# tmr4/T41_SDR

Hardware: AMD Instinct MI355X
Metric: MSamples/s I/Q through full RX chain, batch=4096; achieved HBM GB/s vs roofline (higher is better)
Workload: dtype f32; 1 GPU; configs[1]: batched SSB (USB 200-3000 Hz) RX chain, decimate-by-8 + 512-pt fast-conv + demod + interpolate-by-8, 4096 channels x 2048 complex f32 samples per frame per GPU, per-channel NCO, AGC off, 128 consecutive frames per channel per launch; batch=4096, frame_len=2048, fft_length=512, frames_per_launch=128, buffer_layout=channel-major, world_size_observed=1

## Files before the change

t41_sdr_amd/csrc/rx512_kernel.hpp:

```cpp
#pragma once
#include "rx_chains.hpp"

namespace t41 {

template <int PART, bool AGC = false>
struct Geo {
  static constexpr bool kResident = (PART == 0) && !AGC;
  static constexpr int kWaves = kResident ? 16 : 4;
  static constexpr int kTab = kResident ? 1024 : kLdsTabFloats;
  static constexpr int kTw1 = kResident ? 0 : kLdsTabTw1;
  static constexpr int kTw2 = kResident ? 448 : kLdsTabTw2;
  static constexpr int kSlice = kResident ? 2496 : kLdsFloatsPerWave;
  static constexpr int kTotal = kTab + kWaves * kSlice;
  static constexpr int kX = 0;
  static constexpr int kXF = kResident ? 1348 : kXFloats;
  static constexpr int kY1 = kXF;
  static constexpr int kOV = kY1 + kY1Floats;
  static constexpr int kH1 = kOV + 512;
  static constexpr int kScr = kResident ? 80 : 0;
  static constexpr int kI1 = kScr;
};
template <int MODE, int PART, bool AGC, bool PIPE>
using Rx512Geo = Geo<PART, geo4(MODE, AGC) && !PIPE>;
static_assert(!Geo<0>::kResident || Geo<0>::kTotal * sizeof(float) == 160 * 1024, "PART 0: one workgroup owns the CU's LDS");
static_assert(Geo<1>::kTotal * sizeof(float) == 40960, "PART 1/2: four workgroups per CU");
static_assert(pipe_layout(7).counters == (size_t)7 * kPipeSlots * kPipeSlotFloats * sizeof(float) &&
              pipe_layout(7).timeout == pipe_layout(7).counters + ((size_t)7 + 15) * 16 * sizeof(unsigned long long) &&
              pipe_layout(7).second == pipe_layout(7).counters + ((size_t)7 + 16) * 32 * sizeof(float) && kPipeStatWords == 16,
              "rx512_kernel's pipe_err / pipe_stat / sam_slots arithmetic follows pipe_layout()");
static_assert(!Geo<0>::kResident || (Geo<0>::kH1 + 24 <= Geo<0>::kSlice && Geo<0>::kScr + 8 * kFftRow * 2 <= Geo<0>::kXF &&
                                     Geo<0>::kI1 + 284 <= Geo<0>::kXF && Geo<0>::kScr >= 68), "resident LDS layout");

constexpr int kPartMap = 4;
constexpr int kPartSet = 8;
constexpr int kPartA24 = 16;
constexpr int kPartOut = 32;
template <int MODE, bool DEBUG, int PARTM, bool PLAIN, bool AGC = false, bool WQ15 = false, bool SEGPAR = false, bool PIPE = false>
__global__ __launch_bounds__((Rx512Geo<MODE, (PARTM & 3), AGC, PIPE>::kWaves * 64), 4) void rx512_kernel(const RxArgs a) {
  T41RX_CLK_BEGIN();
  constexpr int PART = PARTM & 3;
  constexpr bool MAP = (PARTM & kPartMap) != 0;
  constexpr bool SET = (PARTM & kPartSet) != 0;
  constexpr bool A24 = (PARTM & kPartA24) != 0;
  constexpr bool OUT = (PARTM & kPartOut) != 0;
  static_assert(PART <= 2 && (PARTM & ~(3 | kPartMap | kPartSet | kPartA24 | kPartOut)) == 0,
                "PARTM = PART, PART + kPartMap, or PART + kPartMap + kPartSet, each of the mapped ones with or without kPartA24 and kPartOut");
  static_assert(!OUT || (MAP && PART == 0 && !DEBUG && !SEGPAR) || ((PARTM & ~kPartSet) == 2 + kPartOut && SEGPAR),
                "the output-map form is a twin of the mapped FFT_LENGTH 512 kernels without taps, and of the segment-parallel back kernel");
  static_assert(!A24 || (MAP && PART == 0 && !DEBUG && !SEGPAR), "the 24 kS/s form is a twin of the mapped FFT_LENGTH 512 kernels without taps");
  static_assert(!SET || (MAP && PART == 0 && !SEGPAR) || (PARTM == 2 + kPartOut + kPartSet && SEGPAR),
                "the set form is a twin of the mapped FFT_LENGTH 512 kernels, and of the back kernel's output-map form");
  static_assert(!MAP || PART != 2, "the back end of the long-FFT pipeline reads no antenna samples");
  static_assert(!SEGPAR || (PART == 1 && MODE != kModeNfm) || (PART == 2 && MODE == kModeSsb && !AGC), "SEGPAR variants");
  static_assert(!PIPE || ((AGC || MODE == kModeSam) && PART == 0 && !DEBUG && !SEGPAR),
                "PIPE: the pipelined variants -- AGC on (see agc_prep_pipe), the synchronous detector with the AGC off (sam_chain_pipe), or both (PSA)");
  constexpr bool PSAM = PIPE && MODE == kModeSam && !AGC;
  constexpr bool PSA = PIPE && MODE == kModeSam && AGC;
  constexpr int kPF = PSAM ? kPrefetchPipeSam : PIPE ? kPrefetchPipe : kPrefetch;
  typedef Rx512Geo<MODE, PART, AGC, PIPE> G;
  constexpr bool KEEP = G::kResident;
  constexpr int NW = G::kWaves;
  constexpr int kX = G::kX, kY1 = G::kY1, kScr = G::kScr, kI1 = G::kI1;
  __shared__ __attribute__((aligned(16))) float smem[G::kTotal];
  constexpr int L = 2048, D = 256, N = 512;
  const int seg = (PART == 0) ? 1 : a.seg;
  const size_t state_stride = state_floats(512 * seg);
  int lane = threadIdx.x & 63;
  const int wv = __builtin_amdgcn_readfirstlane(threadIdx.x >> 6);
  const int job = blockIdx.x * NW + wv;
  const int runs = SEGPAR ? (a.nframes + a.seg_run - 1) / a.seg_run : 1;
  const int ch = SEGPAR ? job / runs : job;
  const int seg0 = SEGPAR ? (job - ch * runs) * a.seg_run : 0;
  const int seg1 = SEGPAR ? (seg0 + a.seg_run < a.nframes ? seg0 + a.seg_run : a.nframes) : a.nframes;

  auto stage_tables = [&]() {
    const float4 *src = reinterpret_cast<const float4 *>(a.tab);
    float4 *dst = reinterpret_cast<float4 *>(smem);
    if (PART == 1) {
      if (threadIdx.x < 128) dst[threadIdx.x] = reinterpret_cast<const float4 *>(a.tab + kTabSinCos)[threadIdx.x];
    } else if (KEEP) {
      if (threadIdx.x < 224) dst[threadIdx.x] = src[kTabTw1 / 2 + threadIdx.x];
      else if (threadIdx.x >= 256 && threadIdx.x < 256 + 56)
        reinterpret_cast<float2 *>(smem)[G::kTw2 + threadIdx.x - 256] =
            a.tab[kTabTw2 + 64 * ((threadIdx.x - 256) >> 3) + ((threadIdx.x - 256) & 7)];
      else if (PIPE && threadIdx.x >= 320 && threadIdx.x < 332)
        reinterpret_cast<unsigned *>(smem)[kPipeFlags + threadIdx.x - 320] = 0u;
    } else if (MODE == kModeSam) {
      for (int i = threadIdx.x; i < 516; i += 256) smem[i] = reinterpret_cast<const float *>(a.tab + kTabSam)[i];
      for (int i = 512 / 2 + threadIdx.x; i < (512 + 448) / 2; i += 256) dst[i] = src[i];
      if (threadIdx.x < 56)
        reinterpret_cast<float2 *>(smem)[kLdsTabTw2 + threadIdx.x] = a.tab[kTabTw2 + 64 * (threadIdx.x >> 3) + (threadIdx.x & 7)];
    } else {
      for (int i = threadIdx.x; i < (512 + 448) / 2; i += 256) dst[i] = src[i];
      if (threadIdx.x < 56)
        reinterpret_cast<float2 *>(smem)[kLdsTabTw2 + threadIdx.x] = a.tab[kTabTw2 + 64 * (threadIdx.x >> 3) + (threadIdx.x & 7)];
    }
    __syncthreads();
  };
  const float2 hp8 = a.tab[kTabHp8 + lane];
  const float2 hp4 = a.tab[kTabHp4 + lane];
  if (ch >= a.nchan) {
    if (PART != 2) stage_tables();
    return;
  }

  const cf *ltab = reinterpret_cast<const cf *>(smem);
  float *lds = smem + G::kTab + wv * G::kSlice;
  float *st = a.state + (size_t)ch * state_stride;
  typedef const __attribute__((address_space(4))) int *MapPtr;
  const int pset = SET ? ((MapPtr)a.set_of)[ch] : 0;
  const CoefPtr cf0 = SET ? (CoefPtr)a.coef + pset : (CoefPtr)a.coef;
  const NcoPtr nco = (NcoPtr)(a.nco + ch);
  const float2 *__restrict__ tab = a.tab;
// ... 669 lines not shown
          wave_sync();
  #pragma unroll
          for (int rd = 0; rd < 2; ++rd) {
            const int m0 = 128 * rd + 2 * lane;
            f2 acc = splat(0.0f);
            float tp[96];
  #pragma unroll
            for (int c = 0; c < 96; c += 16) {
              float chunk[16];
              load_taps<16>(chunk, (CFloatPtr)cf0, kCoDeemph + c);
  #pragma unroll
              for (int k = 0; k < 16; ++k) tp[c + k] = chunk[k];
  #pragma unroll
              for (int jj = c / 2; jj < c / 2 + 8; ++jj) {
                if (2 * jj > kDeemphTaps) continue;
                const float2 w = *reinterpret_cast<const float2 *>(ds + m0 + 2 * jj);
                static_assert(kDeemphTaps == 81, "2 jj <= 80 below: tap 2 jj always exists");
                const float t_m1 = (jj > 0) ? tp[2 * jj - 1] : 0.0f;
                const float t_p1 = (2 * jj + 1 < kDeemphTaps) ? tp[2 * jj + 1] : 0.0f;
                f2 pr = f2{tp[2 * jj], t_m1} * splat(w.x);
                acc = acc + pr;
                pr = f2{t_p1, tp[2 * jj]} * splat(w.y);
                acc = acc + pr;
              }
            }
            au[rd][0] = (m0 < D - kDeemphTaps) ? acc.x : y2[rd][0].y;
            au[rd][1] = (m0 + 1 < D - kDeemphTaps) ? acc.y : y2[rd][1].y;
          }
          wave_sync();
        }
        if (PART == 0) {
          if (lane == 63) *reinterpret_cast<cf *>(st + kStMisc + kMiscNfmI) = y2[0][1];
        } else {
          if (lane == 63 && (f & (seg - 1)) == seg / 2 - 1) *reinterpret_cast<cf *>(st + kStMisc + kMiscNfmI) = y2[1][1];
          nfm_carry = cf{__int_as_float(__builtin_amdgcn_readlane(__float_as_int(y2[1][1].x), 63)),
                         __int_as_float(__builtin_amdgcn_readlane(__float_as_int(y2[1][1].y), 63))};
        }
  #pragma unroll
        for (int rd = 0; rd < 2; ++rd)
  #pragma unroll
          for (int e = 0; e < 2; ++e) y2[rd][e] = cf{au[rd][e], 0.0f};
      }
      if (PART == 1) {
        float *mid = a.mid + ((size_t)ch * a.nframes + f) * (2 * D);
  #pragma unroll
        for (int rd = 0; rd < 2; ++rd)
          *reinterpret_cast<float4 *>(mid + 2 * (128 * rd + 2 * lane)) =
              make_float4(y2[rd][0].x, y2[rd][0].y, y2[rd][1].x, y2[rd][1].y);
        continue;
      }


      {
        cf *tb = reinterpret_cast<cf *>(lds + kScr);
  #pragma unroll
        for (int rd = 0; rd < 2; ++rd)
          *reinterpret_cast<float4 *>(lds + kScr + 2 * (128 * rd + 2 * lane)) =
              make_float4(y2[rd][0].x, y2[rd][0].y, y2[rd][1].x, y2[rd][1].y);
        wave_sync();
  #pragma unroll
        for (int j = 0; j < 4; ++j) v[4 + j] = tb[lane + 64 * j];
        constexpr bool OVL_REAL = MODE == kModeNfm;
        if (KEEP) {
          cf *ov = reinterpret_cast<cf *>(lds + G::kOV);
  #pragma unroll
          for (int j = 0; j < 4; ++j) v[j] = ov[64 * j + lane];
  #pragma unroll
          for (int j = 0; j < 4; ++j) {
            if (OVL_REAL) ov[64 * j + lane].x = v[4 + j].x;
            else ov[64 * j + lane] = v[4 + j];
          }
        } else {
          cf *ov = reinterpret_cast<cf *>(st + kStOverlap);
  #pragma unroll
          for (int j = 0; j < 4; ++j) {
            if (OVL_REAL) ov[64 * j + lane].x = v[4 + j].x;
            else ov[64 * j + lane] = v[4 + j];
          }
        }
        if (OVL_REAL) {
  #pragma unroll
          for (int j = 0; j < 4; ++j) v[j].y = 0.0f;
        }
      }

      STAMP(6);
      FRESH_LANE();
      {
        cf tw1[7], tw2[7];
        cf mk[8];
        constexpr bool GMASK = KEEP || MODE == kModeSam;
        constexpr bool SMASK = SET && !GMASK;
        if (SMASK) {
  #pragma unroll
          for (int r = 0; r < 8; ++r) {
            const float2 t = ptab[kTabMask + 64 * r + lane];
            mk[r] = cf{t.x, t.y};
          }
        }
        if (!GMASK) {
  #pragma unroll
          for (int q = 0; q < 7; ++q) {
            tw1[q] = ltab[G::kTw1 + 64 * q + lane];
            tw2[q] = ltab[G::kTw2 + 8 * q + (lane & 7)];
          }
        }
        if (GMASK) {
          fft512_ldstw<false>(v, ltab + G::kTw1 + lane, ltab + G::kTw2 + (lane & 7), lds + kScr, lane, [&]() {
  #pragma unroll
            for (int r = 0; r < 8; ++r) {
              const float2 t = ptab[kTabMask + 64 * r + lane];
              mk[r] = cf{t.x, t.y};
            }
          });
        } else {
          fft512<false>(v, tw1, tw2, lds + kScr, lane);
        }
  #pragma unroll
        for (int r = 0; r < 8; ++r) v[r] = cmul(v[r], (GMASK || SMASK) ? mk[r] : ltab[kLdsTabMask + 64 * r + lane]);
        if (DEBUG && a.spect_max && tap_row >= 0) {
          float *sp = a.spect ? a.spect + ((size_t)ch * tap_stride + tap_row) * 1024 : nullptr;
          float best = -1.0f;
          int besti = 0;
  #pragma unroll
          for (int r = 0; r < 8; ++r) {
            const int k = lane + 64 * r;
            const float re = v[r].x * 512.0f, im = v[r].y * 512.0f;
            const float e0 = im * im, e1 = re * re;
            if (sp) *reinterpret_cast<float2 *>(sp + 1022 - 2 * k) = make_float2(e0, e1);
            if (e1 >= best) { best = e1; besti = 1023 - 2 * k; }
            if (e0 >= best) { best = e0; besti = 1022 - 2 * k; }
          }
  #pragma unroll
          for (int m = 1; m < 64; m <<= 1) {
            const float ob = __shfl_xor(best, m, 64);
            const int oi = __shfl_xor(besti, m, 64);
            if (ob > best || (ob == best && oi < besti)) { best = ob; besti = oi; }
          }
          if (lane == 0) {
            float *mx = a.spect_max + ((size_t)ch * tap_stride + tap_row) * 3;
            const float ave = (float)(.5 * (double)best + .5 * (double)st[kStMisc + kMiscMaxSqAve]);
            mx[0] = best;
            mx[1] = (float)besti;
            mx[2] = ave;
            st[kStMisc + kMiscMaxSqAve] = ave;
          }
        }
        if (GMASK)
          fft512_ldstw<true>(v, ltab + G::kTw1 + lane, ltab + G::kTw2 + (lane & 7), lds + kScr, lane, []() {});
        else
          fft512<true>(v, tw1, tw2, lds + kScr, lane);
      }
    }
    FRESH_LANE();
    if (PART != 2 || LONGC) {
      const float fixed_gain = fresh_coef(cf0)->sc[kScFixedGain];
      cf og[4];
      if (PSA) {
        const int left = a.nchan - NW * (int)blockIdx.x;
        const int nvalid = left < NW ? left : NW;
        unsigned *fa = reinterpret_cast<unsigned *>(smem) + kPipeFlags;
        unsigned *fs = fa + 5;
        unsigned *pipe_err = reinterpret_cast<unsigned *>(reinterpret_cast<unsigned long long *>(a.agc_pipe + (size_t)a.nchan * kPipeSlots * kPipeSlotFloats) +
                                                          ((size_t)a.nchan + 15) * 16);
        float *sam_slots = a.agc_pipe + (size_t)a.nchan * kPipeSlots * kPipeSlotFloats + ((size_t)a.nchan + 16) * 32;
        const size_t ch0 = (size_t)NW * blockIdx.x;
        auto claim = [&](unsigned *word, int g) -> bool {
          unsigned won = 0u;
          if (lane == 0) {
            unsigned expect = (unsigned)g;
            won = __hip_atomic_compare_exchange_strong(word, &expect, (unsigned)(g + 1), __ATOMIC_RELAXED, __ATOMIC_RELAXED, __HIP_MEMORY_SCOPE_WORKGROUP) ? 1u : 0u;
          }
          return __builtin_amdgcn_readfirstlane(won) != 0u;
        };
        static_assert(!PSA || (NW == 16 && kScr + kPipeStageFloats <= G::kXF && kScr + kPipeSamStageFloats <= G::kXF), "chain staging inside the X scratch");
        if (f < seg1) {
          float *pslot = a.agc_pipe + ((size_t)ch * kPipeSlots + f % kPipeSlots) * kPipeSlotFloats;
          if (first_iter) agmag = make_float2(agc_mag(cf{agrec.x, agrec.y}), agc_mag(cf{agrec.z, agrec.w}));
          agrec = agc_prep_pipe<AgcLds<true>, true>(v, agrec, agmag, lds, pslot, cf0, lane);
          __builtin_amdgcn_fence(__ATOMIC_RELEASE, "workgroup");
          if (lane == 0) __hip_atomic_fetch_add(fa + f % kPipeSlots, 1u, __ATOMIC_RELAXED, __HIP_MEMORY_SCOPE_WORKGROUP);
        }
        {
          const int g = f - 1;
          if (g >= seg0 && g < seg1 && claim(fa + 4, g)) {
            pipe_wait_ge(fa + g % kPipeSlots, (unsigned)nvalid, pipe_err);
            if (lane == 0) __hip_atomic_store(fa + g % kPipeSlots, 0u, __ATOMIC_RELAXED, __HIP_MEMORY_SCOPE_WORKGROUP);
            PRIO(3);
            unsigned long long *pipe_stat = reinterpret_cast<unsigned long long *>(a.agc_pipe + (size_t)a.nchan * kPipeSlots * kPipeSlotFloats) + (size_t)job * 16;
            agc_chain_pipe(a.agc_pipe + (ch0 * kPipeSlots + g % kPipeSlots) * kPipeSlotFloats, a.state + ch0 * state_stride + st_agc(512) + kAgcHistFloats,
                           state_stride, lds + kScr, fa + 3, (unsigned)g, nvalid, chain_coef, lane, pipe_stat, pipe_err);
            PRIO(1);
            __builtin_amdgcn_fence(__ATOMIC_RELEASE, "workgroup");
            if (lane == 0) __hip_atomic_store(fa + 3, (unsigned)(g + 1), __ATOMIC_RELAXED, __HIP_MEMORY_SCOPE_WORKGROUP);
          }
        }
        {
          const int fm = f - 2;
          if (fm >= seg0 && fm < seg1) {
            pipe_wait_ge(fa + 3, (unsigned)(fm + 1), pipe_err);
            __builtin_amdgcn_fence(__ATOMIC_ACQUIRE, "workgroup");
            const AgcGainIn gin = agc_gain_request<true>(a.agc_pipe + ((size_t)ch * kPipeSlots + fm % kPipeSlots) * kPipeSlotFloats, lane);
// ... 337 lines not shown
        hist1c = lds4(lds + kI1 + 256 + 4 * lane);
        if (!SEGPAR || (seg0 == 0 && seg1 == a.nframes)) *reinterpret_cast<float4 *>(st + kStInt1 + 4 * lane) = hist1c;
      }
#pragma unroll
      for (int u = 0; u < 4; ++u) u1[u] = splat(0.0f);
#pragma unroll
      for (int b = 0; b < 24; b += 8) {
        float ci[16];
        load_taps<16>(ci, (CFloatPtr)cf0, kCoInt1 + 2 * b);
#pragma unroll
        for (int u = 0; u < 4; ++u) {
#pragma unroll
          for (int t = 0; t < 8; ++t) u1[u] = pk_fma(splat(w[u + b + t + 1]), f2{ci[1 + 2 * t], ci[2 * t]}, u1[u]);
        }
      }
    }
    STAMP(11);
    FRESH_LANE();
    {
      float w[15];
      float c4[32];
      load_taps<32>(c4, (CFloatPtr)cf0, kCoInt2);
      const float x1[8] = {u1[0].x, u1[0].y, u1[1].x, u1[1].y, u1[2].x, u1[2].y, u1[3].x, u1[3].y};
#pragma unroll
      for (int i = 0; i < 7; ++i) {
        const float up = lane_up1(x1[i + 1]);
        const float hs = __int_as_float(__builtin_amdgcn_readlane(__float_as_int(hist2), i + 1));
        w[i] = write_lane<0>(up, hs);
      }
#pragma unroll
      for (int i = 0; i < 8; ++i) w[7 + i] = x1[i];
      if (!KEEP && lane == 63 && (!SEGPAR || (seg0 == 0 && seg1 == a.nframes))) {
        *reinterpret_cast<float4 *>(st + kStInt2) = make_float4(0.0f, x1[1], x1[2], x1[3]);
        *reinterpret_cast<float4 *>(st + kStInt2 + 4) = make_float4(x1[4], x1[5], x1[6], x1[7]);
      }
      if (PART == 2 && SEGPAR && seg0 == 0 && f == seg1 - 1 && seg1 < a.nframes) {
        const float *end = a.aud24 + ((size_t)ch * a.nframes + a.nframes) * D;
        if (lane < 6) *reinterpret_cast<float4 *>(st + kStInt1 + 4 * lane) = *reinterpret_cast<const float4 *>(end - 24 + 4 * lane);
        float xp[8];
        x2_tail(end, xp);
        if (lane == 0) {
          *reinterpret_cast<float4 *>(st + kStInt2) = make_float4(0.0f, xp[1], xp[2], xp[3]);
          *reinterpret_cast<float4 *>(st + kStInt2 + 4) = make_float4(xp[4], xp[5], xp[6], xp[7]);
        }
      }
      if (PART == 2 || KEEP) {
  #define T41RX_HIST2_ENTRY(i) hist2c = write_lane<i>(hist2c, __int_as_float(__builtin_amdgcn_readlane(__float_as_int(x1[i]), 63)));
        T41RX_HIST2_ENTRY(1) T41RX_HIST2_ENTRY(2) T41RX_HIST2_ENTRY(3) T41RX_HIST2_ENTRY(4) T41RX_HIST2_ENTRY(5) T41RX_HIST2_ENTRY(6) T41RX_HIST2_ENTRY(7)
  #undef T41RX_HIST2_ENTRY
      }
      wave_sync();
      unsigned qw[2] = {0u, 0u};
      constexpr bool PARK = KEEP && !WQ15;
      constexpr int kOvPark = (2048 - G::kOV + 3) / 4;
      static_assert(!PARK || (kOvPark > 0 && kOvPark <= 64 && G::kH1 >= 2048), "parking layout");
      float4 park_h = any_float4(), park_o = any_float4();
      if (PARK) {
        if (lane < 14) park_h = lds4(lds + kX + 2 * xpad(2 * lane));
        else if (lane >= 16 && lane < 40) park_h = lds4(lds + kY1 + y1slot(lane - 16));
        if (lane < kOvPark) park_o = lds4(lds + G::kOV + 4 * lane);
        wave_sync();
      }
      float *tr = PARK ? lds : lds + kScr;
#pragma unroll
      for (int u = 0; u < 8; ++u) {
        f2 o01 = splat(0.0f), o23 = splat(0.0f);
#pragma unroll
        for (int t = 0; t < 8; ++t) {
          const f2 x = splat(w[u + t]);
          o01 = pk_fma(x, f2{c4[4 * t + 3], c4[4 * t + 2]}, o01);
          o23 = pk_fma(x, f2{c4[4 * t + 1], c4[4 * t]}, o23);
        }
        if (!WQ15) {
          *reinterpret_cast<float4 *>(tr + 4 * (8 * lane + (u ^ (lane & 7)))) = make_float4(o01.x, o01.y, o23.x, o23.y);
        } else if ((u & 1) == 0) {
          qw[0] = q15_pack2(o01.x, o01.y);
          qw[1] = q15_pack2(o23.x, o23.y);
        } else {
          const int piece = u >> 1;
          *reinterpret_cast<uint4 *>(tr + 4 * (4 * lane + (piece ^ ((lane >> 1) & 3)))) =
              make_uint4(qw[0], qw[1], q15_pack2(o01.x, o01.y), q15_pack2(o23.x, o23.y));
        }
      }
      wave_sync();
      STAMP(12);
      if (!WQ15) {
        const LaneOff lof = fresh_off(4 * lane);
#pragma unroll
        for (int i = 0; i < 8; ++i) {
          const int row = 8 * i + (lane >> 3);
          const float4 t = lds4(tr + 4 * (8 * row + ((lane & 7) ^ (row & 7))));
          stg_stream(gO + 256 * i, lof, t);
        }
      } else {
        const LaneOff lof = fresh_off(4 * lane);
#pragma unroll
        for (int i = 0; i < 4; ++i) {
          const int row = 16 * i + (lane >> 2);
          const float4 t = lds4(tr + 4 * (4 * row + ((lane & 3) ^ ((row >> 1) & 3))));
          stg_stream(gO + 256 * i, lof, t);
        }
      }
      if (PARK) {
        wave_sync();
        if (lane < 14) *reinterpret_cast<float4 *>(lds + kX + 2 * xpad(2 * lane)) = park_h;
        else if (lane >= 16 && lane < 40) *reinterpret_cast<float4 *>(lds + kY1 + y1slot(lane - 16)) = park_h;
        if (lane < kOvPark) *reinterpret_cast<float4 *>(lds + G::kOV + 4 * lane) = park_o;
      }
    }
    STAMP(13);
#ifdef T41RX_PIPE_STAT
    if (PIPE && lane == 0)
      (reinterpret_cast<unsigned long long *>(a.agc_pipe + (size_t)a.nchan * kPipeSlots * kPipeSlotFloats) + (size_t)job * 16)[10] += __builtin_readcyclecounter() - ps_t;
#endif
  }
#ifdef T41RX_STAMP
  {
    unsigned long long rt;
    asm volatile("s_memrealtime %0\n\ts_waitcnt lgkmcnt(0)" : "=s"(rt)::"memory");
    if (lane == 29) stamp_acc = rt;
  }
  if (a.dbg_demod && PART != 2)
    reinterpret_cast<unsigned long long *>(a.dbg_demod + (size_t)a.nchan * a.nframes * D)[(size_t)ch * 64 + lane] = stamp_acc;
#endif

  if (PIPE && AGC && lane < 50) *reinterpret_cast<float4 *>(st + st_agc(512) + 4 * lane) = agrec;
  if (KEEP) {
    wave_sync();
    if (lane < 14) *reinterpret_cast<float4 *>(st + kStDec1 + 4 * lane) = lds4(lds + kX + 2 * xpad(2 * lane));
    if (lane < 24) *reinterpret_cast<float4 *>(st + kStDec2 + 4 * lane) = lds4(lds + kY1 + y1slot(lane));
    *reinterpret_cast<float4 *>(st + kStOverlap + 4 * lane) = lds4(lds + G::kOV + 4 * lane);
    *reinterpret_cast<float4 *>(st + kStOverlap + 256 + 4 * lane) = lds4(lds + G::kOV + 256 + 4 * lane);
    if (!A24 && !muted) {
      if (lane < 6) *reinterpret_cast<float4 *>(st + kStInt1 + 4 * lane) = lds4(lds + G::kH1 + 4 * lane);
      if (lane < 8) st[kStInt2 + lane] = (lane == 0) ? 0.0f : hist2c;
    }
  }
  if (PART != 2 && lane == 0) {
    if (!SEGPAR || seg0 == 0) {
      ncs->phase = phase0;
      ncs->r = osc_r;
      st[kStMisc + kMiscDc] = dc_carry;
    }
  }
  T41RX_CLK_END(job);
}

}
```

t41_sdr_amd/csrc/rx_device.hpp:

```cpp
#pragma once
#include <hip/hip_runtime.h>

#include <cstdlib>

#include "rx_experiments.hpp"
#include "rx_internal.hpp"
#include "rx_kernels.hpp"
#include "wave_fft.hpp"


namespace t41 {

constexpr int kPrefetch = 2;
constexpr int kPrefetchPipe = 0;
constexpr int kPrefetchPipeSam = 1;

#define PRIO(n) __builtin_amdgcn_s_setprio(n)
#define FRESH_LANE() asm volatile("" : "+v"(lane))
#define FRESH_WV(w) asm volatile("" : "+s"(w))

#ifdef T41RX_STAMP
#define STAMP(p)                                                                     \
  do {                                                                               \
    unsigned long long t_;                                                           \
    __builtin_amdgcn_sched_barrier(0);                                               \
    asm volatile("s_memtime %0\n\ts_waitcnt lgkmcnt(0)" : "=s"(t_)::"memory"); \
    __builtin_amdgcn_sched_barrier(0);                                               \
    if (lane == (p)) stamp_acc += t_ - stamp_last;                                   \
    stamp_last = t_;                                                                 \
  } while (0)
#define STAMP_PARAMS , unsigned long long &stamp_acc, unsigned long long &stamp_last
#define STAMP_ARGS , stamp_acc, stamp_last
#else
#define STAMP(p) do {} while (0)
#define STAMP_PARAMS
#define STAMP_ARGS
#endif

template <bool INV, typename MID>
__device__ __forceinline__ void fft512_ldstw(cf (&v)[8], const cf *tw1l, const cf *tw2l, float *__restrict__ xbuf,
                                             int lane, MID mid) {
  cf *xb = reinterpret_cast<cf *>(xbuf);
  dft8<INV>(v);
#pragma unroll
  for (int q = 1; q < 8; ++q) {
    const cf w = tw1l[64 * (q - 1)];
    v[q] = INV ? cmulc(v[q], w) : cmul(v[q], w);
  }
  fft_exchange1_perm(v);
  mid();
  dft8<INV>(v);
#pragma unroll
  for (int q = 1; q < 8; ++q) {
    const cf w = tw2l[8 * (q - 1)];
    v[q] = INV ? cmulc(v[q], w) : cmul(v[q], w);
  }
  wave_sync();
  {
    const int l1 = lane & 7, q = lane >> 3;
#pragma unroll
    for (int q2 = 0; q2 < 8; ++q2) xb[q2 * kFftRow + q + fft_x2(l1)] = v[q2];
  }
  wave_sync();
  {
    const int q = lane & 7, q2 = lane >> 3;
#pragma unroll
    for (int l1 = 0; l1 < 8; ++l1) v[l1] = xb[q2 * kFftRow + q + fft_x2(l1)];
  }
  dft8<INV>(v);
}

template <bool INV>
__device__ __forceinline__ void fft512_ldstw_x2(cf (&v)[8], cf (&u)[8], const cf *tw1l, const cf *tw2l,
                                                float *__restrict__ xbuf_v, float *__restrict__ xbuf_u, int lane) {
  cf *xv = reinterpret_cast<cf *>(xbuf_v), *xu = reinterpret_cast<cf *>(xbuf_u);
  const int l1 = lane & 7, q3 = lane >> 3;
  dft8<INV>(v);
  dft8<INV>(u);
#pragma unroll
  for (int q = 1; q < 8; ++q) {
    const cf w = tw1l[64 * (q - 1)];
    v[q] = INV ? cmulc(v[q], w) : cmul(v[q], w);
    u[q] = INV ? cmulc(u[q], w) : cmul(u[q], w);
  }
  fft_exchange1_perm(v);
  fft_exchange1_perm(u);
  dft8<INV>(v);
  dft8<INV>(u);
#pragma unroll
  for (int q = 1; q < 8; ++q) {
    const cf w = tw2l[8 * (q - 1)];
    v[q] = INV ? cmulc(v[q], w) : cmul(v[q], w);
    u[q] = INV ? cmulc(u[q], w) : cmul(u[q], w);
  }
  wave_sync();
#pragma unroll
  for (int q2 = 0; q2 < 8; ++q2) xv[q2 * kFftRow + q3 + fft_x2(l1)] = v[q2];
#pragma unroll
  for (int q2 = 0; q2 < 8; ++q2) xu[q2 * kFftRow + q3 + fft_x2(l1)] = u[q2];
  wave_sync();
#pragma unroll
  for (int j = 0; j < 8; ++j) v[j] = xv[q3 * kFftRow + l1 + fft_x2(j)];
#pragma unroll
  for (int j = 0; j < 8; ++j) u[j] = xu[q3 * kFftRow + l1 + fft_x2(j)];
  dft8<INV>(v);
  dft8<INV>(u);
}

constexpr double kHpB0 = 0.927176191943378969;
constexpr double kHpB1 = -0.927176191943378969;
constexpr double kHpA1 = 0.854352383886757938;
constexpr double cpow(double b, int e) {
  double r = 1.0;
  for (int i = 0; i < e; ++i) r *= b;
  return r;
}
template <int n>
struct HpTab {
  float scanA[4];
  float pw[n];
  constexpr HpTab() : scanA{}, pw{} {
    for (int s = 0; s < 4; ++s) scanA[s] = (float)cpow(kHpA1, n << s);
// ... 115 lines not shown
#pragma clang diagnostic pop
}
typedef float f4n __attribute__((ext_vector_type(4)));
__device__ __forceinline__ float4 ldg_stream(const float *p) {
  const f4n t = __builtin_nontemporal_load(reinterpret_cast<const f4n *>(p));
  return make_float4(t.x, t.y, t.z, t.w);
}
__device__ __forceinline__ void stg_stream(float *p, float4 v) {
  __builtin_nontemporal_store(f4n{v.x, v.y, v.z, v.w}, reinterpret_cast<f4n *>(p));
}
struct LaneOff {
  unsigned bytes;
};
__device__ __forceinline__ LaneOff fresh_off(int floats) {
  unsigned o = (unsigned)floats * 4u;
  asm volatile("" : "+v"(o));
  return LaneOff{o};
}
typedef __attribute__((address_space(1))) char *GlobalBytes;
typedef const __attribute__((address_space(1))) char *CGlobalBytes;
typedef const __attribute__((address_space(1))) f4n *CGlobalF4;
typedef __attribute__((address_space(1))) f4n *GlobalF4;
__device__ __forceinline__ CGlobalBytes global_at(const float *ubase, LaneOff o) {
  CGlobalBytes b = (CGlobalBytes)(ubase);
  asm("" : "+s"(b));
  return b + o.bytes;
}
__device__ __forceinline__ GlobalBytes global_at(float *ubase, LaneOff o) {
  GlobalBytes b = (GlobalBytes)(ubase);
  asm("" : "+s"(b));
  return b + o.bytes;
}
__device__ __forceinline__ float4 ldg_stream(const float *ubase, LaneOff o, int imm = 0) {
  const f4n t = __builtin_nontemporal_load((CGlobalF4)(global_at(ubase, o) + 4 * imm));
  return make_float4(t.x, t.y, t.z, t.w);
}
__device__ __forceinline__ void stg_stream(float *ubase, LaneOff o, float4 v) {
  __builtin_nontemporal_store(f4n{v.x, v.y, v.z, v.w}, (GlobalF4)global_at(ubase, o));
}
__device__ __forceinline__ float2 ldg2(const float2 *ubase, unsigned idx) {
  typedef float f2n __attribute__((ext_vector_type(2)));
  CGlobalBytes b = (CGlobalBytes)(ubase);
  asm("" : "+s"(b));
  unsigned o = idx * 8u;
  asm volatile("" : "+v"(o));
  const f2n t = *(const __attribute__((address_space(1))) f2n *)(b + o);
  return make_float2(t.x, t.y);
}
__device__ __forceinline__ f2 ldg_cf(const f2 *ubase, LaneOff o, int imm = 0) {
  typedef float f2n __attribute__((ext_vector_type(2)));
  const f2n t = *(const __attribute__((address_space(1))) f2n *)(global_at(reinterpret_cast<const float *>(ubase), o) + 8 * imm);
  return f2{t.x, t.y};
}
__device__ __forceinline__ float4 ldg4(const float *ubase, LaneOff o) {
  const f4n t = *(CGlobalF4)global_at(ubase, o);
  return make_float4(t.x, t.y, t.z, t.w);
}

__device__ __forceinline__ float q15_lo(float w) { return (float)(short)(__float_as_uint(w) & 0xffffu); }
__device__ __forceinline__ float q15_hi(float w) { return (float)(__float_as_int(w) >> 16); }
__device__ __forceinline__ unsigned q15_pack2(float x0, float x1) {
  int a = (int)(x0 * 32768.0f), b = (int)(x1 * 32768.0f);
  a = a < -32768 ? -32768 : (a > 32767 ? 32767 : a);
  b = b < -32768 ? -32768 : (b > 32767 ? 32767 : b);
  return ((unsigned)a & 0xffffu) | ((unsigned)b << 16);
}

typedef float f4v __attribute__((ext_vector_type(4)));
typedef float f8v __attribute__((ext_vector_type(8)));
typedef float f16v __attribute__((ext_vector_type(16)));
typedef const __attribute__((address_space(4))) float *CFloatPtr;
constexpr int kCoDec1 = offsetof(DevCoef, dec1) / 4, kCoDec2 = offsetof(DevCoef, dec2) / 4, kCoInt1 = offsetof(DevCoef, int1) / 4,
              kCoInt2 = offsetof(DevCoef, int2) / 4, kCoDeemph = offsetof(DevCoef, deemph) / 4;
template <int N>
__device__ __forceinline__ void load_taps(float (&dst)[N], CFloatPtr base, int off) {
  asm volatile("" : "+s"(base));
  const CFloatPtr p = base + off;
  static_assert(N % 4 == 0, "tap chunks are multiples of 4");
  int i = 0;
#pragma unroll
  for (; i + 16 <= N; i += 16) {
    const f16v t = *reinterpret_cast<const __attribute__((address_space(4))) f16v *>(p + i);
#pragma unroll
    for (int j = 0; j < 16; ++j) dst[i + j] = t[j];
  }
#pragma unroll
  for (; i + 8 <= N; i += 8) {
    const f8v t = *reinterpret_cast<const __attribute__((address_space(4))) f8v *>(p + i);
#pragma unroll
    for (int j = 0; j < 8; ++j) dst[i + j] = t[j];
  }
#pragma unroll
  for (; i + 4 <= N; i += 4) {
    const f4v t = *reinterpret_cast<const __attribute__((address_space(4))) f4v *>(p + i);
#pragma unroll
    for (int j = 0; j < 4; ++j) dst[i + j] = t[j];
  }
}

__device__ __forceinline__ cf fir_mac(float tap, cf x, cf acc) {
  return pk_fma(splat(tap), x, acc);
}
template <int NT, int OFF0, int OFF1, int NLOAD, int GROUP, int TAIL0 = 1 << 20, typename IDX>
__device__ __forceinline__ void fir_pair(const float *win, IDX idx, CoefPtr coef, int taps, cf &acc0, cf &acc1,
                                         const cf *tail = nullptr) {
  constexpr int NTP = (NT + 7) & ~7;
  float tc[NTP];
  acc0 = splat(0.0f);
// ... 64 lines not shown
```

t41_sdr_amd/csrc/rx_host.cpp:

```cpp
#include <hip/hip_runtime.h>

#include <cmath>
#include <cstdio>
#include <cstdlib>
#include <cstring>
#include <memory>
#include <new>
#include <string>
#include <utility>
#include <vector>

#include "rx_ctx.hpp"

using namespace t41;

namespace {
thread_local std::string g_last_error;
}

int t41::fail(int code, const std::string &msg) {
  g_last_error = msg;
  return code;
}

// ... 62 lines not shown
  f.nfm_atan = p.mode == T41RX_DEMOD_NFM && p.nfm_demod == 1;
  f.plain_gains = plain_gains;
  f.nr = p.nrOptionSelect != 0 || p.ANR_notchOn != 0;
  return f;
}

bool t41::gains_of(const float *sc, SetGains &g) {
  const bool iq_on = sc[kScIqCorrOn] != 0.0f;
  const float gi = iq_on ? sc[kScBandGain] * sc[kScNegIqAmp] : sc[kScBandGain];
  g = SetGains{};
  g.g_rf = sc[kScRfGain];
  g.g_band = sc[kScBandGain];
  g.neg_iq_amp = sc[kScNegIqAmp];
  g.iq_phase = sc[kScIqPhase];
  g.iq_corr_on = iq_on ? 1 : 0;
  return (iq_on ? gi == -1.0f : gi == 1.0f) && sc[kScBandGain] == 1.0f && (!iq_on || sc[kScIqPhase] == 0.0f);
}

namespace {
int upload_coeffs(t41rx_ctx *ctx) {
  const int N = ctx->params.fft_length;
  BlobView v = blob_view(ctx->blob.data());
  DevCoef dc;
  fill_dev_coef(v, dc);
  HIP_TRY(hipMemcpy(ctx->d_coef.get(), &dc, sizeof(dc), hipMemcpyHostToDevice));

  const int R = N / 512;
  std::vector<float2> tab;
  fill_tab512(v, N, tab);
  const float invN = 1.0f / (float)N;
  if (N != 512) {
    std::vector<float2> t4((size_t)tab_long_entries(R));
    const double tp = 6.283185307179586476925286766559;
    for (int q = 1; q < R; ++q)
      for (int k = 0; k < 512; ++k) {
        const double a = -tp * (double)(k * q) / (double)N;
        t4[(size_t)(512 * (q - 1) + k)] = make_float2((float)std::cos(a), (float)std::sin(a));
      }
    for (int q = 0; q < R; ++q)
      for (int m = 0; m < 512; ++m) {
        const int k = q + R * m;
        t4[(size_t)((R - 1) * 512 + 512 * q + m)] = make_float2(v.mask[2 * k] * invN, v.mask[2 * k + 1] * invN);
      }
    HIP_TRY(hipMemcpy(ctx->d_tab4k.get(), t4.data(), sizeof(float2) * t4.size(), hipMemcpyHostToDevice));
  }
  HIP_TRY(hipMemcpy(ctx->d_tab.get(), tab.data(), sizeof(float2) * tab.size(), hipMemcpyHostToDevice));
  return T41RX_OK;
}
}

void t41::fill_tab512(const BlobView &v, int N, std::vector<float2> &tab) {
  tab.assign((size_t)kTabEntries512, make_float2(0.0f, 0.0f));
  const float invN = 1.0f / (float)N;
  if (N == 512) {
    for (int r = 0; r < 8; ++r)
      for (int l = 0; l < 64; ++l) {
        const int k = l + 64 * r;
        tab[(size_t)(kTabMask + 64 * r + l)] = make_float2(v.mask[2 * k] * invN, v.mask[2 * k + 1] * invN);
      }
  }
  const double two_pi = 6.283185307179586476925286766559;
  for (int q = 1; q < 8; ++q)
    for (int l = 0; l < 64; ++l) {
      const double a1 = -two_pi * (double)(l * q) / 512.0;
      const double a2 = -two_pi * (double)((l & 7) * q) / 64.0;
      tab[(size_t)(kTabTw1 + 64 * (q - 1) + l)] = make_float2((float)std::cos(a1), (float)std::sin(a1));
      tab[(size_t)(kTabTw2 + 64 * (q - 1) + l)] = make_float2((float)std::cos(a2), (float)std::sin(a2));
    }
  for (int i = 0; i < 256; ++i) {
    const double a = two_pi * (double)i / 256.0;
    tab[(size_t)(kTabSinCos + i)] = make_float2((float)std::cos(a), (float)std::sin(a));
  }
  for (int l = 0; l < 64; ++l) {
    const double a1 = 0.854352383886757938;
    tab[(size_t)(kTabHp8 + l)] = make_float2((float)std::pow(a1, 8.0 * ((l & 15) + 1)), (float)std::pow(a1, 8.0 * ((l & 31) + 1)));
    tab[(size_t)(kTabHp4 + l)] = make_float2((float)std::pow(a1, 4.0 * ((l & 15) + 1)), (float)std::pow(a1, 4.0 * ((l & 31) + 1)));
  }
  {
    const double ca = (double)0.99f, a4 = ca * ca * ca * ca;
    struct M2 { float a, b, c, d; };
    auto mm = [](M2 x, M2 y) { return M2{x.a * y.a + x.b * y.c, x.a * y.b + x.b * y.d, x.c * y.a + x.d * y.c, x.c * y.b + x.d * y.d}; };
    const M2 M{v.lp1[3], v.lp1[4], 1.0f, 0.0f};
    const M2 Mq = mm(M, M), P1 = mm(Mq, Mq);
    for (int l = 0; l < 64; ++l) {
      double p15 = a4, p31 = a4;
      M2 Q15 = P1, Q31 = P1;
      for (int i = 0; i < (l & 15); ++i) { p15 *= a4; Q15 = mm(Q15, P1); }
      for (int i = 0; i < (l & 31); ++i) { p31 *= a4; Q31 = mm(Q31, P1); }
      float2 *e = &tab[(size_t)(kTabAm + 6 * l)];
      std::memcpy(&e[0], &p15, sizeof(double));
      std::memcpy(&e[1], &p31, sizeof(double));
      e[2] = make_float2(Q15.a, Q15.b);
      e[3] = make_float2(Q15.c, Q15.d);
      e[4] = make_float2(Q31.a, Q31.b);
      e[5] = make_float2(Q31.c, Q31.d);
    }
  }
  {
    float *t = reinterpret_cast<float *>(&tab[(size_t)kTabSam]);
    for (int k = 0; k <= 512; ++k) t[k] = (float)std::sin(6.283185307179586476925286766559 * (double)k / 512.0);
    t[0] = 0.0f;
    t[256] = 0.0f;
    t[512] = -0.0f;
  }
}

namespace {

int pipe_timeouts(const t41rx_ctx *ctx) {
  if (!ctx->d_agc_pipe) return 0;
  unsigned n = 0;
  if (hipMemcpy(&n, ctx->d_agc_pipe.get() + pipe_layout(ctx->nchan).timeout, sizeof(n), hipMemcpyDeviceToHost) != hipSuccess)
    return -1;
// ... 636 lines not shown
```

t41_sdr_amd/csrc/rx_internal.hpp:

```cpp
#pragma once
#include <cstddef>
#include <cstdint>

#include "../../include/t41rx.h"

namespace t41 {

constexpr int kSampleRate = 192000;
constexpr int kDec1Taps = 28;
constexpr int kDec2Taps = 46;
constexpr int kInt1Taps = 48;
constexpr int kInt2Taps = 32;

constexpr uint32_t kBlobMagic = 0x54343152u;
constexpr int kBlobParamInts = 24;
constexpr int kBlobHeaderInts = 8 + kBlobParamInts;
static_assert(sizeof(t41rx_params) <= kBlobParamInts * sizeof(int32_t), "params section of the blob header");
constexpr int kNumScalars = 16;
enum Scalar {
  kScRfGain = 0,
  kScBandGain = 1,
  kScNegIqAmp = 2,
  kScIqPhase = 3,
  kScLevel = 4,
  kScFixedGain = 5,
  kScOutScale = 6,
  kScIqCorrOn = 7,
  kScSideTone = 8,
  kScNfmDemod = 9,
  kScSamWmin = 10,
  kScSamWmax = 11,
  kScSamG1 = 12,
  kScSamG2 = 13,
};
constexpr int kDeemphTaps = 81;
extern const float kDeemphFir24000[kDeemphTaps];
constexpr int kNumAgc = 16;
enum AgcConst {
  kAgcAttackMult = 0, kAgcDecayMult, kAgcFastDecayMult, kAgcFastBackmult, kAgcOnemFastBackmult,
  kAgcHangBackmult, kAgcOnemHangBackmult, kAgcHangDecayMult, kAgcOutTarget, kAgcMinVolts,
  kAgcSlopeConstant, kAgcInvMaxInput, kAgcHangLevel, kAgcPopRatio,
  kAgcHangCount,
  kAgcAttackBuffsize,
};
struct BlobView {
  int32_t *header;
  float *dec1, *dec2, *int1, *int2, *lp1, *scalars, *agc, *mask;
};
constexpr size_t blob_floats(int fft_length) {
  return kBlobHeaderInts + kDec1Taps + kDec2Taps + kInt1Taps + kInt2Taps + 5 + kNumScalars + kNumAgc +
         2 * (size_t)fft_length;
}
inline BlobView blob_view(void *blob) {
  BlobView v;
  v.header = reinterpret_cast<int32_t *>(blob);
  float *f = reinterpret_cast<float *>(blob) + kBlobHeaderInts;
  v.dec1 = f;
  v.dec2 = v.dec1 + kDec1Taps;
  v.int1 = v.dec2 + kDec2Taps;
  v.int2 = v.int1 + kInt1Taps;
  v.lp1 = v.int2 + kInt2Taps;
  v.scalars = v.lp1 + 5;
  v.agc = v.scalars + kNumScalars;
  v.mask = v.agc + kNumAgc;
  return v;
}

extern const float kZoomIirCoeffs[4][20];
void design_zoom_fir(int spectrumZoom, float (&coeffs)[4]);
constexpr int kDispIir = 0;
constexpr int kDispFir = 32;
constexpr int kDispPtr = 40;
constexpr int kDispRing = 64;
constexpr int kDispOld = 64 + 1024;
constexpr int kDispFloats = kDispOld + 512;
constexpr int kCalPixel = kDispFloats;
constexpr int kCalFloats = kCalPixel + 256;
constexpr int kPanPixel = kDispFloats;
constexpr int kPanOldNf = kPanPixel + 256;
constexpr int kPanNewSpectrum = kPanOldNf + 1;
constexpr int kPanFloats = kPanOldNf + 4;
constexpr int kPanGradient = 117;
inline int pan_rows_of_call(long long counter, int n_frames, int period, int phase, int *first) {
  const int f0 = (int)((((long long)phase - counter) % period + period) % period);
  *first = f0 < n_frames ? f0 : n_frames;
  return f0 < n_frames ? (n_frames - 1 - f0) / period + 1 : 0;
}

int design_blob(const t41rx_params &p, void *blob, size_t blob_bytes);
bool params_valid(const t41rx_params &p, const char **why);
void nr_vad_range(int FLoCut, int FHiCut, int *lo, int *hi);

struct DevCoef {
  float dec1[kDec1Taps];
  float dec2[48];
  float int1[kInt1Taps];
  float int2[kInt2Taps];
  float lp1[8];
  float sc[16];
  float agc[16];
  float deemph[96];
};

struct ChanNco {
  uint64_t phase_inc;
  float wk[8][2];
  double r_star_sq;
  double w_abs;
};
static_assert(sizeof(ChanNco) == 8 + 64 + 16, "ChanNco layout");

constexpr int kStDec1 = 0;
constexpr int kStDec2 = 56;
constexpr int kStInt1 = 152;
constexpr int kStInt2 = 176;
constexpr int kStMisc = 184;
constexpr int kMiscDc = 0;
constexpr int kMiscWold = 2;
// ... 36 lines not shown
```

t41_sdr_amd/csrc/rx_kernels.hpp:

```cpp
#pragma once
#include <hip/hip_runtime.h>

#include "rx_internal.hpp"
#include "rx_plan.hpp"

namespace t41 {

constexpr int kTabMask = 0;
constexpr int kTabTw1 = 512;
constexpr int kTabTw2 = kTabTw1 + 7 * 64;
constexpr int kTabSinCos = kTabTw2 + 7 * 64;
constexpr int kTabHp8 = kTabSinCos + 256;
constexpr int kTabHp4 = kTabHp8 + 64;
constexpr int kTabAm = kTabHp4 + 64;
constexpr int kTabSam = kTabAm + 64 * 6;
constexpr int kTabEntries512 = kTabSam + 260;

struct SetGains {
  float g_rf, g_band, neg_iq_amp, iq_phase;
  int iq_corr_on;
  int pad[3];
};
static_assert(sizeof(SetGains) == 32, "SetGains: one 32-byte scalar load");

struct RxArgs {
  const float *__restrict__ I;
  const float *__restrict__ Q;
  float *__restrict__ out;
  float *__restrict__ state;
  const DevCoef *__restrict__ coef;
  const float2 *__restrict__ tab;
  const ChanNco *__restrict__ nco;
  int nchan;
  int nframes;
  long long chan_stride;
  long long frame_stride;
  float *dbg_nco;
  float *dbg_dec;
  float *dbg_demod;
  float *dbg_pre;
  float *spect;
  float *spect_max;
  float *mid;
  float *aud24;
  const float2 *tab4k;
  int nframes4k;
  int seg;
  int plain;
  int agc;
  float g_rf;
  float g_band;
  float neg_iq_amp;
  float iq_phase;
  int iq_corr_on;
  int q15;
  int nfm_atan;
  int seg_run;
  int ovl_real;
  int nco_rd;
  float *aud_out;
  float *agc_pipe;
  const int *__restrict__ in_map;
  long long in_chan_stride;
  long long in_frame_stride;
  int tap_period;
  int tap_first;
  int tap_rows;
  const int *__restrict__ set_of;
  const SetGains *__restrict__ set_gain;
// ... 86 lines not shown
```

t41_sdr_amd/csrc/wave_fft.hpp:

```cpp
#pragma once
#include <hip/hip_runtime.h>

namespace t41 {

__device__ __forceinline__ void wave_sync() {
  asm volatile("" ::: "memory");
  __builtin_amdgcn_wave_barrier();
  __builtin_amdgcn_sched_barrier(0);
  asm volatile("" ::: "memory");
}


typedef float f2 __attribute__((ext_vector_type(2)));
typedef f2 cf;

__device__ __forceinline__ f2 splat(float s) { return f2{s, s}; }
__device__ __forceinline__ f2 pk_fma(f2 a, f2 b, f2 c) { return __builtin_elementwise_fma(a, b, c); }

__device__ __forceinline__ cf cmul(cf a, cf b) {
  cf t, r;
  asm("v_pk_mul_f32 %0, %1, %2 op_sel:[1,1] op_sel_hi:[1,0] neg_lo:[0,1]" : "=v"(t) : "v"(a), "v"(b));
  asm("v_pk_fma_f32 %0, %1, %2, %3 op_sel:[0,0,0] op_sel_hi:[0,1,1]" : "=v"(r) : "v"(a), "v"(b), "v"(t));
  return r;
}
__device__ __forceinline__ cf cmulc(cf a, cf b) {
  cf t, r;
  asm("v_pk_mul_f32 %0, %1, %2 op_sel:[1,1] op_sel_hi:[1,0]" : "=v"(t) : "v"(a), "v"(b));
  asm("v_pk_fma_f32 %0, %1, %2, %3 op_sel:[0,0,0] op_sel_hi:[0,1,1] neg_hi:[0,1,0]" : "=v"(r) : "v"(a), "v"(b), "v"(t));
  return r;
}
__device__ __forceinline__ cf cmul_s(cf a, cf b_uniform) {
  cf t, r;
  asm("v_pk_mul_f32 %0, %1, %2 op_sel:[1,1] op_sel_hi:[1,0] neg_lo:[0,1]" : "=v"(t) : "v"(a), "s"(b_uniform));
  asm("v_pk_fma_f32 %0, %1, %2, %3 op_sel:[0,0,0] op_sel_hi:[0,1,1]" : "=v"(r) : "v"(a), "s"(b_uniform), "v"(t));
  return r;
}
__device__ __forceinline__ cf add_mj(cf a, cf b) {
  cf r;
  asm("v_pk_add_f32 %0, %1, %2 op_sel:[0,1] op_sel_hi:[1,0] neg_hi:[0,1]" : "=v"(r) : "v"(a), "v"(b));
  return r;
}
__device__ __forceinline__ cf add_pj(cf a, cf b) {
  cf r;
  asm("v_pk_add_f32 %0, %1, %2 op_sel:[0,1] op_sel_hi:[1,0] neg_lo:[0,1]" : "=v"(r) : "v"(a), "v"(b));
  return r;
}

template <bool INV>
__device__ __forceinline__ void dft8(cf (&v)[8]) {
  constexpr float kR = 0.70710678118654752440f;
  const cf a0 = v[0] + v[4], a1 = v[0] - v[4];
  const cf a2 = v[2] + v[6], a3 = v[2] - v[6];
  const cf a4 = v[1] + v[5], a5 = v[1] - v[5];
  const cf a6 = v[3] + v[7], a7 = v[3] - v[7];
  const cf b0 = a0 + a2, b1 = a0 - a2;
  const cf b2 = a4 + a6, b3 = a4 - a6;
  const cf c0 = INV ? add_pj(a1, a3) : add_mj(a1, a3);
  const cf c1 = INV ? add_mj(a1, a3) : add_pj(a1, a3);
  const cf d0 = INV ? add_pj(a5, a7) : add_mj(a5, a7);
  const cf d1 = INV ? add_mj(a5, a7) : add_pj(a5, a7);
  const cf t0 = INV ? add_pj(d0, d0) : add_mj(d0, d0);
  const cf t1 = INV ? add_mj(d1, d1) : add_pj(d1, d1);
  v[0] = b0 + b2;
  v[4] = b0 - b2;
  v[2] = INV ? add_pj(b1, b3) : add_mj(b1, b3);
  v[6] = INV ? add_mj(b1, b3) : add_pj(b1, b3);
  v[1] = pk_fma(t0, splat(kR), c0);
  v[5] = pk_fma(t0, splat(-kR), c0);
  v[3] = pk_fma(t1, splat(-kR), c1);
  v[7] = pk_fma(t1, splat(kR), c1);
}

constexpr int kFftRow = 72;
__device__ __forceinline__ constexpr int fft_x2(int l1) { return 8 * l1 + (l1 & 6); }

__device__ __forceinline__ void lane_swap32(float &a, float &b) {
  const auto r = __builtin_amdgcn_permlane32_swap(__float_as_uint(a), __float_as_uint(b), false, false);
  a = __uint_as_float(r[0]);
  b = __uint_as_float(r[1]);
}
__device__ __forceinline__ void lane_swap16(float &a, float &b) {
  const auto r = __builtin_amdgcn_permlane16_swap(__float_as_uint(a), __float_as_uint(b), false, false);
  a = __uint_as_float(r[0]);
  b = __uint_as_float(r[1]);
}
__device__ __forceinline__ void lane_swap8(float &a, float &b) {
  const float t = b;
  b = __int_as_float(__builtin_amdgcn_update_dpp(__float_as_int(b), __float_as_int(a), 0x108 , 0xf, 0x3, false));
  a = __int_as_float(__builtin_amdgcn_update_dpp(__float_as_int(a), __float_as_int(t), 0x118 , 0xf, 0xc, false));
}
__device__ __forceinline__ void fft_exchange1_perm(cf (&v)[8]) {
  float re[8], im[8];
#pragma unroll
  for (int q = 0; q < 8; ++q) {
    re[q] = v[q].x;
    im[q] = v[q].y;
  }
#pragma unroll
  for (int q = 0; q < 4; ++q) {
    lane_swap32(re[q], re[q + 4]);
    lane_swap32(im[q], im[q + 4]);
  }
#pragma unroll
  for (int q = 0; q < 8; ++q) {
    if (q & 2) continue;
    lane_swap16(re[q], re[q + 2]);
    lane_swap16(im[q], im[q + 2]);
  }
#pragma unroll
  for (int q = 0; q < 8; q += 2) {
    lane_swap8(re[q], re[q + 1]);
    lane_swap8(im[q], im[q + 1]);
  }
#pragma unroll
  for (int q = 0; q < 8; ++q) v[q] = cf{re[q], im[q]};
}


template <bool INV>
__device__ __forceinline__ void fft512(cf (&v)[8], const cf (&tw1)[7], const cf (&tw2)[7],
                                       float *__restrict__ xbuf, int lane) {
  cf *xb = reinterpret_cast<cf *>(xbuf);
  dft8<INV>(v);
// ... 44 lines not shown
```

Before: 405,700 MSamples/s.

## Trim resident SSB path: single-buffer overlap, paired mask loads, real-only upper inverse DFT

For the resident, non-pipelined, non-NFM kernel, the overlap buffer is read once and then overwritten in place, which removes the separate scratch round-trip. The filter mask is now read as 16-byte paired loads from a new interleaved table section. The final inverse radix-8 stage computes only the real parts of the upper outputs that SSB demod consumes. Register parking collapses to a single float4 per lane at a computed LDS address. Together these cut LDS traffic, load instructions and ALU work, in exchange for a larger table and layout constraints enforced by static asserts.

```diff
diff --git a/t41_sdr_amd/csrc/rx512_kernel.hpp b/t41_sdr_amd/csrc/rx512_kernel.hpp
--- a/t41_sdr_amd/csrc/rx512_kernel.hpp
+++ b/t41_sdr_amd/csrc/rx512_kernel.hpp
@@ -59,6 +59,7 @@
   constexpr int kPF = PSAM ? kPrefetchPipeSam : PIPE ? kPrefetchPipe : kPrefetch;
   typedef Rx512Geo<MODE, PART, AGC, PIPE> G;
   constexpr bool KEEP = G::kResident;
+  constexpr bool LEAN = KEEP && !PIPE && MODE != kModeNfm;
   constexpr int NW = G::kWaves;
   constexpr int kX = G::kX, kY1 = G::kY1, kScr = G::kScr, kI1 = G::kI1;
   __shared__ __attribute__((aligned(16))) float smem[G::kTotal];
@@ -834,16 +835,23 @@
 
 
       {
-        cf *tb = reinterpret_cast<cf *>(lds + kScr);
+        constexpr bool OVL_REAL = MODE == kModeNfm;
+        constexpr bool OVL_ONCE = LEAN;
+        cf *tb = reinterpret_cast<cf *>(lds + (OVL_ONCE ? G::kOV : kScr));
+        if (OVL_ONCE) {
+  #pragma unroll
+          for (int j = 0; j < 4; ++j) v[j] = tb[64 * j + lane];
+          wave_sync();
+        }
   #pragma unroll
         for (int rd = 0; rd < 2; ++rd)
-          *reinterpret_cast<float4 *>(lds + kScr + 2 * (128 * rd + 2 * lane)) =
+          *reinterpret_cast<float4 *>(reinterpret_cast<float *>(tb) + 2 * (128 * rd + 2 * lane)) =
               make_float4(y2[rd][0].x, y2[rd][0].y, y2[rd][1].x, y2[rd][1].y);
         wave_sync();
   #pragma unroll
         for (int j = 0; j < 4; ++j) v[4 + j] = tb[lane + 64 * j];
-        constexpr bool OVL_REAL = MODE == kModeNfm;
-        if (KEEP) {
+        if (OVL_ONCE) {
+        } else if (KEEP) {
           cf *ov = reinterpret_cast<cf *>(lds + G::kOV);
   #pragma unroll
           for (int j = 0; j < 4; ++j) v[j] = ov[64 * j + lane];
@@ -873,6 +881,7 @@
         cf mk[8];
         constexpr bool GMASK = KEEP || MODE == kModeSam;
         constexpr bool SMASK = SET && !GMASK;
+        constexpr bool PMASK = LEAN && !DEBUG;
         if (SMASK) {
   #pragma unroll
           for (int r = 0; r < 8; ++r) {
@@ -889,10 +898,20 @@
         }
         if (GMASK) {
           fft512_ldstw<false>(v, ltab + G::kTw1 + lane, ltab + G::kTw2 + (lane & 7), lds + kScr, lane, [&]() {
-  #pragma unroll
-            for (int r = 0; r < 8; ++r) {
-              const float2 t = ptab[kTabMask + 64 * r + lane];
-              mk[r] = cf{t.x, t.y};
+            if (PMASK) {
+              const LaneOff lof = fresh_off(2 * kTabMask2 + 4 * lane);
+  #pragma unroll
+              for (int q = 0; q < 4; ++q) {
+                const float4 t = ldg4(reinterpret_cast<const float *>(ptab), lof, 256 * q);
+                mk[2 * q] = cf{t.x, t.y};
+                mk[2 * q + 1] = cf{t.z, t.w};
+              }
+            } else {
+  #pragma unroll
+              for (int r = 0; r < 8; ++r) {
+                const float2 t = ptab[kTabMask + 64 * r + lane];
+                mk[r] = cf{t.x, t.y};
+              }
             }
           });
         } else {
@@ -928,8 +947,9 @@
             st[kStMisc + kMiscMaxSqAve] = ave;
           }
         }
+        constexpr bool RE_HI = KEEP && MODE == kModeSsb && !AGC && !DEBUG;
         if (GMASK)
-          fft512_ldstw<true>(v, ltab + G::kTw1 + lane, ltab + G::kTw2 + (lane & 7), lds + kScr, lane, []() {});
+          fft512_ldstw<true, RE_HI>(v, ltab + G::kTw1 + lane, ltab + G::kTw2 + (lane & 7), lds + kScr, lane, []() {});
         else
           fft512<true>(v, tw1, tw2, lds + kScr, lane);
       }
@@ -1373,16 +1393,28 @@
       wave_sync();
       unsigned qw[2] = {0u, 0u};
       constexpr bool PARK = KEEP && !WQ15;
-      constexpr int kOvPark = (2048 - G::kOV + 3) / 4;
-      static_assert(!PARK || (kOvPark > 0 && kOvPark <= 64 && G::kH1 >= 2048), "parking layout");
+      constexpr bool PARK1 = PARK && LEAN;
+      constexpr int kTrW = PARK1 ? 68 : 0;
+      constexpr int kOvPark = (kTrW + 2048 - G::kOV + 3) / 4;
+      static_assert(!PARK || (kOvPark > 0 && kOvPark <= 64 && G::kH1 >= kTrW + 2048), "parking layout");
+      static_assert(!PARK1 || (kTrW >= 2 * xpad(26) + 4 && kTrW % 4 == 0 && kTrW <= kY1 && kY1 + y1slot(1) + 48 <= G::kOV &&
+                               G::kOV >= kTrW && 24 + kOvPark == 64), "one-register parking: the /4 history outside, 64 float4 of state inside");
       float4 park_h = any_float4(), park_o = any_float4();
-      if (PARK) {
+      static_assert(y1slot(1) - 48 == 256 && G::kOV - 96 == kY1 + 512, "the parked pieces lie 256 + 48 floats apart");
+      const auto park_at = [](int l) {
+        const unsigned r = ((unsigned)l * 11u) >> 7;
+        return kY1 + 4 * l + 256 * (int)(r < 2u ? r : 2u);
+      };
+      if (PARK1) {
+        park_h = lds4(lds + park_at(lane));
+        wave_sync();
+      } else if (PARK) {
         if (lane < 14) park_h = lds4(lds + kX + 2 * xpad(2 * lane));
         else if (lane >= 16 && lane < 40) park_h = lds4(lds + kY1 + y1slot(lane - 16));
         if (lane < kOvPark) park_o = lds4(lds + G::kOV + 4 * lane);
         wave_sync();
       }
-      float *tr = PARK ? lds : lds + kScr;
+      float *tr = PARK ? lds + kTrW : lds + kScr;
 #pragma unroll
       for (int u = 0; u < 8; ++u) {
         f2 o01 = splat(0.0f), o23 = splat(0.0f);
@@ -1422,7 +1454,11 @@
           stg_stream(gO + 256 * i, lof, t);
         }
       }
-      if (PARK) {
+      if (PARK1) {
+        wave_sync();
+        FRESH_LANE();
+        *reinterpret_cast<float4 *>(lds + park_at(lane)) = park_h;
+      } else if (PARK) {
         wave_sync();
         if (lane < 14) *reinterpret_cast<float4 *>(lds + kX + 2 * xpad(2 * lane)) = park_h;
         else if (lane >= 16 && lane < 40) *reinterpret_cast<float4 *>(lds + kY1 + y1slot(lane - 16)) = park_h;
diff --git a/t41_sdr_amd/csrc/rx_device.hpp b/t41_sdr_amd/csrc/rx_device.hpp
--- a/t41_sdr_amd/csrc/rx_device.hpp
+++ b/t41_sdr_amd/csrc/rx_device.hpp
@@ -37,7 +37,7 @@
 #define STAMP_ARGS
 #endif
 
-template <bool INV, typename MID>
+template <bool INV, bool RE_HI = false, typename MID>
 __device__ __forceinline__ void fft512_ldstw(cf (&v)[8], const cf *tw1l, const cf *tw2l, float *__restrict__ xbuf,
                                              int lane, MID mid) {
   cf *xb = reinterpret_cast<cf *>(xbuf);
@@ -67,7 +67,8 @@
 #pragma unroll
     for (int l1 = 0; l1 < 8; ++l1) v[l1] = xb[q2 * kFftRow + q + fft_x2(l1)];
   }
-  dft8<INV>(v);
+  if constexpr (RE_HI) dft8_re_hi<INV>(v);
+  else dft8<INV>(v);
 }
 
 template <bool INV>
@@ -289,8 +290,8 @@
   const f2n t = *(const __attribute__((address_space(1))) f2n *)(global_at(reinterpret_cast<const float *>(ubase), o) + 8 * imm);
   return f2{t.x, t.y};
 }
-__device__ __forceinline__ float4 ldg4(const float *ubase, LaneOff o) {
-  const f4n t = *(CGlobalF4)global_at(ubase, o);
+__device__ __forceinline__ float4 ldg4(const float *ubase, LaneOff o, int imm = 0) {
+  const f4n t = *(CGlobalF4)(global_at(ubase, o) + 4 * imm);
   return make_float4(t.x, t.y, t.z, t.w);
 }
 
diff --git a/t41_sdr_amd/csrc/rx_host.cpp b/t41_sdr_amd/csrc/rx_host.cpp
--- a/t41_sdr_amd/csrc/rx_host.cpp
+++ b/t41_sdr_amd/csrc/rx_host.cpp
@@ -138,13 +138,7 @@
 void t41::fill_tab512(const BlobView &v, int N, std::vector<float2> &tab) {
   tab.assign((size_t)kTabEntries512, make_float2(0.0f, 0.0f));
   const float invN = 1.0f / (float)N;
-  if (N == 512) {
-    for (int r = 0; r < 8; ++r)
-      for (int l = 0; l < 64; ++l) {
-        const int k = l + 64 * r;
-        tab[(size_t)(kTabMask + 64 * r + l)] = make_float2(v.mask[2 * k] * invN, v.mask[2 * k + 1] * invN);
-      }
-  }
+  if (N == 512) fill_tab512_mask(v.mask, invN, reinterpret_cast<float *>(tab.data()));
   const double two_pi = 6.283185307179586476925286766559;
   for (int q = 1; q < 8; ++q)
     for (int l = 0; l < 64; ++l) {
diff --git a/t41_sdr_amd/csrc/rx_internal.hpp b/t41_sdr_amd/csrc/rx_internal.hpp
--- a/t41_sdr_amd/csrc/rx_internal.hpp
+++ b/t41_sdr_amd/csrc/rx_internal.hpp
@@ -64,6 +64,29 @@
   v.agc = v.scalars + kNumScalars;
   v.mask = v.agc + kNumAgc;
   return v;
+}
+
+constexpr int kTabMask = 0;
+constexpr int kTabTw1 = 512;
+constexpr int kTabTw2 = kTabTw1 + 7 * 64;
+constexpr int kTabSinCos = kTabTw2 + 7 * 64;
+constexpr int kTabHp8 = kTabSinCos + 256;
+constexpr int kTabHp4 = kTabHp8 + 64;
+constexpr int kTabAm = kTabHp4 + 64;
+constexpr int kTabSam = kTabAm + 64 * 6;
+constexpr int kTabMask2 = kTabSam + 260;
+constexpr int kTabEntries512 = kTabMask2 + 512;
+static_assert(kTabMask2 % 2 == 0 && kTabEntries512 % 2 == 0, "the paired mask is read 16 bytes at a time, in every set's table");
+inline void fill_tab512_mask(const float *mask, float invN, float *tab) {
+  for (int r = 0; r < 8; ++r)
+    for (int l = 0; l < 64; ++l) {
+      const int k = l + 64 * r;
+      const float re = mask[2 * k] * invN, im = mask[2 * k + 1] * invN;
+      float *one = tab + 2 * (kTabMask + 64 * r + l);
+      float *two = tab + 2 * (kTabMask2 + 2 * (64 * (r >> 1) + l) + (r & 1));
+      one[0] = two[0] = re;
+      one[1] = two[1] = im;
+    }
 }
 
 extern const float kZoomIirCoeffs[4][20];
diff --git a/t41_sdr_amd/csrc/rx_kernels.hpp b/t41_sdr_amd/csrc/rx_kernels.hpp
--- a/t41_sdr_amd/csrc/rx_kernels.hpp
+++ b/t41_sdr_amd/csrc/rx_kernels.hpp
@@ -6,15 +6,6 @@
 
 namespace t41 {
 
-constexpr int kTabMask = 0;
-constexpr int kTabTw1 = 512;
-constexpr int kTabTw2 = kTabTw1 + 7 * 64;
-constexpr int kTabSinCos = kTabTw2 + 7 * 64;
-constexpr int kTabHp8 = kTabSinCos + 256;
-constexpr int kTabHp4 = kTabHp8 + 64;
-constexpr int kTabAm = kTabHp4 + 64;
-constexpr int kTabSam = kTabAm + 64 * 6;
-constexpr int kTabEntries512 = kTabSam + 260;
 
 struct SetGains {
   float g_rf, g_band, neg_iq_amp, iq_phase;
diff --git a/t41_sdr_amd/csrc/wave_fft.hpp b/t41_sdr_amd/csrc/wave_fft.hpp
--- a/t41_sdr_amd/csrc/wave_fft.hpp
+++ b/t41_sdr_amd/csrc/wave_fft.hpp
@@ -69,6 +69,27 @@
   v[5] = pk_fma(t0, splat(-kR), c0);
   v[3] = pk_fma(t1, splat(-kR), c1);
   v[7] = pk_fma(t1, splat(kR), c1);
+}
+
+template <bool INV>
+__device__ __forceinline__ void dft8_re_hi(cf (&v)[8]) {
+  constexpr float kR = 0.70710678118654752440f;
+  const float a0x = v[0].x + v[4].x, a1x = v[0].x - v[4].x;
+  const float a2x = v[2].x + v[6].x, a3y = v[2].y - v[6].y;
+  const cf a4 = v[1] + v[5], a5 = v[1] - v[5];
+  const cf a6 = v[3] + v[7], a7 = v[3] - v[7];
+  const float b0x = a0x + a2x, b1x = a0x - a2x;
+  const float b2x = a4.x + a6.x, b3y = a4.y - a6.y;
+  const float c0x = INV ? a1x - a3y : a1x + a3y;
+  const float c1x = INV ? a1x + a3y : a1x - a3y;
+  const cf d0 = INV ? add_pj(a5, a7) : add_mj(a5, a7);
+  const cf d1 = INV ? add_mj(a5, a7) : add_pj(a5, a7);
+  const float t0x = INV ? d0.x - d0.y : d0.x + d0.y;
+  const float t1x = INV ? d1.x + d1.y : d1.x - d1.y;
+  v[4] = cf{b0x - b2x, 0.0f};
+  v[6] = cf{INV ? b1x + b3y : b1x - b3y, 0.0f};
+  v[5] = cf{__builtin_fmaf(t0x, -kR, c0x), 0.0f};
+  v[7] = cf{__builtin_fmaf(t1x, kR, c1x), 0.0f};
 }
 
 constexpr int kFftRow = 72;
```

Measured after the change: 406,800 MSamples/s, median of 6. No clear change (+0.3%).
